# ratschlab/secedo

Hardware: AMD Instinct MI355X
Metric: cell-pair x locus updates/sec (similarity matrix) (higher is better)
Workload: dtype int64; 1 GPU; C3: 8000 cells x 100000 loci; entries=24345058, kept_entries=24223307, reads=23997029, block_cells=128, tiles=2016, normalization=ADD_MIN, max_fragment_length=1000, num_threads=8, parallelism=single GPU, backend=none, world_size=1, rccl_world_size=1

## Files before the change

secedo_amd/csrc/simmat_api.cpp:

```cpp
#include "simmat_handle.hpp"

#include <algorithm>
#include <cstdio>
#include <new>
#include <utility>

using namespace secedo::host;

namespace {

void note_pileup(secedo_simmat *h, uint32_t n_chr, uint64_t n_loci, uint64_t n_entries, const void *read_ids) {
    Fnv1a id;
    for (uint64_t v : {(uint64_t)n_chr, n_loci, n_entries, (uint64_t)reinterpret_cast<uintptr_t>(read_ids)}) id.add(v);
    h->pileup_identity = id.id();
    if (h->override_identity != h->pileup_identity) {
        if (h->pair_bound_override || h->max_shared_override) h->override_dropped = true;
        h->pair_bound_override = 0;
        h->max_shared_override = 0;
        h->override_identity = 0;
    }
}

int check_pileup_args(const secedo_simmat *h, const void *chr_locus_off, const void *locus_entry_off,
                      const void *id_base16, const void *id_base32, const void *group_id_to_pos, uint32_t n_groups) {
    if (!h) return fail(SECEDO_E_INVALID_ARG, "handle is null");
    if (!chr_locus_off || !locus_entry_off) return fail(SECEDO_E_INVALID_ARG, "null offset arrays");
    if ((id_base16 != nullptr) == (id_base32 != nullptr))
        return fail(SECEDO_E_INVALID_ARG, "exactly one of id_base16 / id_base32 must be given");
    if (!group_id_to_pos && n_groups) return fail(SECEDO_E_INVALID_ARG, "group_id_to_pos is null");
    return SECEDO_OK;
}


struct HostPileupStore {
    std::vector<uint32_t> chr, pos, rid, g2p, idb32;
    std::vector<uint64_t> off;
    std::vector<uint16_t> idb16;
};
int fetch_pileup_to_host(const secedo::DeviceFlatPileup &d, hipStream_t s, HostPileupStore *store,
                         secedo::FlatPileupView *v) {
    SECEDO_TRY(hipStreamSynchronize(s));
    auto fetch = [](auto &to, const void *d_src, size_t n) {
        to.resize(n);
        return n ? hipMemcpy(to.data(), d_src, n * sizeof(to[0]), hipMemcpyDeviceToHost) : hipSuccess;
    };
    SECEDO_TRY(fetch(store->chr, d.chr_locus_off, (size_t)d.n_chr + 1));
    SECEDO_TRY(fetch(store->pos, d.locus_pos, d.n_loci));
    SECEDO_TRY(fetch(store->off, d.locus_entry_off, (size_t)d.n_loci + 1));
    SECEDO_TRY(fetch(store->rid, d.read_ids, d.n_entries));
    SECEDO_TRY(fetch(store->g2p, d.group_id_to_pos, d.n_groups));
    if (d.id_base16) SECEDO_TRY(fetch(store->idb16, d.id_base16, d.n_entries));
    else SECEDO_TRY(fetch(store->idb32, d.id_base32, d.n_entries));
    static const uint16_t none16 = 0;
    static const uint32_t none32 = 0;
    *v = secedo::FlatPileupView{store->chr.data(), d.n_chr, store->pos.data(), store->off.data(), store->rid.data(),
                                d.id_base16 ? (store->idb16.empty() ? &none16 : store->idb16.data()) : nullptr,
                                d.id_base16 ? nullptr : (store->idb32.empty() ? &none32 : store->idb32.data()),
                                store->g2p.data(), d.n_groups};
    return SECEDO_OK;
}

int adopt_host_packing(secedo::PackedPileup &from, secedo::DevicePacked *pk) {
    SECEDO_TRY(pk->blk_off.upload(from.blk_off));
    SECEDO_TRY(pk->entry32.upload(from.entry32));
    SECEDO_TRY(pk->mask32.upload(from.mask32));
    SECEDO_TRY(pk->entry.upload(from.entry));
    SECEDO_TRY(pk->entry_read.upload(from.entry_read));
    SECEDO_TRY(pk->range_off.upload(from.range_off));
    SECEDO_TRY(pk->read_off.upload(from.read_off));
    SECEDO_TRY(pk->read_locus.upload(from.read_locus));
    SECEDO_TRY(pk->read_base.upload(from.read_base));
    pk->num_cells = from.num_cells;
    pk->block_cells = from.block_cells;
    pk->num_blocks = from.num_blocks;
    pk->num_loci = from.num_loci;
    pk->num_entries = from.num_entries;
    pk->num_reads = from.num_reads;
    pk->pair_bound = from.pair_bound;
    pk->cell_sq = nullptr;
    pk->cell_sq_n = 0;
    pk->cell_sq_host = std::move(from.cell_sq);
    pk->multi_entries = from.multi_entries;
    pk->max_read_entries = from.max_read_entries;
    pk->n_wide = from.n_wide;
    pk->stage_masks = from.stage_masks;
    pk->count_tile = from.count_tile;
    pk->cap_entries = from.cap_entries;
    pk->cap_loci = from.cap_loci;
    pk->num_ranges = static_cast<uint32_t>(from.range_off.size()) - 1;
    return SECEDO_OK;
}

struct PrepareArgs {
    uint32_t num_cells, max_fragment_length, num_threads, block_cells;
    bool allow_count_tile;
    int mode;
};

int pack_on_device(secedo_simmat *h, const PrepareArgs &p, hipStream_t s, bool *need_host) {
    if (h->have_host) SECEDO_TRY(upload_flat_pileup(h->view, h->raw, &h->dview));
    const std::string err = secedo::pack_pileup_device(h->dview, p.num_cells, p.max_fragment_length, p.num_threads,
                                                       p.block_cells, &secedo::stage_geometry, p.allow_count_tile, s,
                                                       &h->pk, need_host);
    if (!err.empty()) {
        h->have_host = h->have_device = false;
        return fail(err.find("hip") == 0 ? SECEDO_E_HIP : SECEDO_E_INVALID_ARG, err);
    }
    if (*need_host && p.mode == 2) {
        h->have_host = h->have_device = false;
        return fail(SECEDO_E_LIMIT, "this pileup needs the host packing path (a read is longer than "
                                    "max_fragment_length, or a size limit of the device path)");
    }
    if (!*need_host) h->used_device_packing = 1;
    return SECEDO_OK;
}

int pack_on_host(secedo_simmat *h, const PrepareArgs &p, hipStream_t s) {
    HostPileupStore store;
    secedo::FlatPileupView v = h->view;
    if (!h->have_host) SECEDO_CALL(fetch_pileup_to_host(h->dview, s, &store, &v));
    secedo::PackedPileup packed;
    const std::string err = secedo::pack_pileup(v, p.num_cells, p.max_fragment_length, p.num_threads, p.block_cells,
                                                &secedo::stage_geometry, p.allow_count_tile, &packed);
    if (!err.empty()) {
        h->have_host = h->have_device = false;
        return fail(SECEDO_E_INVALID_ARG, err);
    }
    return adopt_host_packing(packed, &h->pk);
}

int build_tile_table(secedo_simmat *h) {
    const uint32_t nb = h->pk.num_blocks;
    if (h->num_tiles == nb * (nb + 1) / 2 && h->tile_row.p) return SECEDO_OK;
    h->num_tiles = nb * (nb + 1) / 2;
    std::vector<uint16_t> trow, tcol;
    trow.reserve(h->num_tiles);
    tcol.reserve(h->num_tiles);
    for (uint32_t i = 0; i < nb; ++i) {
        for (uint32_t j = i; j < nb; ++j) {
            trow.push_back(static_cast<uint16_t>(i));
            tcol.push_back(static_cast<uint16_t>(j));
        }
    }
    SECEDO_TRY(h->tile_row.upload(trow));
    SECEDO_TRY(h->tile_col.upload(tcol));
    h->host_tile_row = trow;
    h->host_tile_col = tcol;
    return SECEDO_OK;
}

int build_flag_lists(secedo_simmat *h, hipStream_t s) {
    const secedo::DevicePacked &pk = h->pk;
    if (!(pk.count_tile && !pk.stage_masks && pk.num_entries)) return SECEDO_OK;
    const uint32_t ne = (uint32_t)pk.num_entries;
    const size_t n_off = (size_t)pk.num_blocks * (pk.num_loci + 1);
    SECEDO_TRY(h->flag_tmp.ensure(secedo::flag_list_scratch_bytes(ne)));
    SECEDO_TRY(h->flag_rec.ensure((size_t)ne * 16));
    SECEDO_TRY(h->flag_idx.ensure((size_t)ne * 4));
    SECEDO_TRY(h->flag_grp.ensure(std::max<size_t>(n_off, 1) * 4));
    SECEDO_TRY(secedo::pack_flag_lists(pk.entry32.as<uint32_t>(), pk.entry.as<uint4>(), ne, pk.blk_off.as<uint32_t>(),
                                       n_off, h->flag_tmp.p, h->flag_grp.as<uint32_t>(), h->flag_rec.as<uint4>(),
                                       h->flag_idx.as<uint32_t>(), s));
    h->flags_ready = true;
    return SECEDO_OK;
}

int print_stamps(secedo_simmat *h) {
    const unsigned long long *counters = h->counters.as<unsigned long long>();
    const bool counts = env_set("SECEDO_STAMPS_COUNTS");
    unsigned long long st[16] = {0};
    SECEDO_TRY(hipMemcpy(st, counters, sizeof(st), hipMemcpyDeviceToHost));
    if (counts) {
        unsigned long long cf[11] = {0};
        SECEDO_TRY(hipMemcpy(cf, counters + 82, sizeof(cf), hipMemcpyDeviceToHost));
        if (cf[0])
            std::fprintf(stderr, "[stamps-correct] pair tests %llu, tail terms %llu, joint terms %llu, later-locus pairs %llu | "
                                 "per wave: pairs phase %.0f cycles (%.0f until the first q records are there), flush phase %.0f cycles, "
                                 "flagged row entries %.0f; busiest lane: %.1f q iterations, %.0f cycles until their records are there\n",
                         cf[0], cf[1], cf[2], cf[3], (double)cf[4] / (double)cf[6], (double)cf[8] / (double)cf[6],
                         (double)cf[5] / (double)cf[6], (double)cf[7] / (double)cf[6], (double)cf[10] / (double)cf[6],
                         (double)cf[9] / (double)cf[6]);
    }
    if (st[8] && counts) {
        const double w = (double)st[8];
        std::fprintf(stderr, "[stamps-counts] sampled waves %llu | per wave cycles: total %.0f barrier-A %.0f stage+barrier-B %.0f "
                             "items(+col prefetch issue) %.0f primary groups %.0f drain %.0f | per primary batch %.0f, per drain batch %.0f "
                             "(%.2f drain batches per primary batch)\n",
                     st[8], st[7] / w, st[2] / w, st[3] / w, st[4] / w, st[5] / w, st[6] / w,
                     (double)st[5] / std::max<double>(1, (double)st[9]), (double)st[6] / std::max<double>(1, (double)st[10]),
                     (double)st[10] / std::max<double>(1, (double)st[9]));
        unsigned long long pw[64] = {0};
        SECEDO_TRY(hipMemcpy(pw, counters + 16, sizeof(pw), hipMemcpyDeviceToHost));
        const double wgs = w / 16.0;
        for (int k = 0; k < 16; ++k)
            std::fprintf(stderr, "[stamps-counts] wave %2d: barrier-A %8.0f  pairs %8.0f  items %8.0f  stage+B %8.0f\n", k,
                         pw[k * 4] / wgs, pw[k * 4 + 1] / wgs, pw[k * 4 + 2] / wgs, pw[k * 4 + 3] / wgs);
    } else if (st[8]) {
        std::fprintf(stderr, "[stamps] waves %llu batches %llu trips %llu | per wave: lifetime %.0f cyc, setup %.0f, "
                             "fill %.0f, trips %.0f | per batch: setup %.0f fill %.0f trips %.0f (%.2f trips)\n",
                     st[8], st[5], st[6], (double)st[7] / st[8], (double)st[2] / st[8], (double)st[3] / st[8],
                     (double)st[4] / st[8], (double)st[2] / st[5], (double)st[3] / st[5], (double)st[4] / st[5],
                     (double)st[6] / st[5]);
        std::fprintf(stderr, "[stamps] per wave: barrier-1 wait %.0f, staging+barrier-2 %.0f, prefetch issue %.0f\n",
                     (double)st[9] / st[8], (double)st[10] / st[8], (double)st[11] / st[8]);
        std::fprintf(stderr, "[stamps] per wave: post-trip %.0f, batch loop total %.0f\n",
                     (double)st[12] / st[8], (double)st[13] / st[8]);
        std::fprintf(stderr, "[stamps] longest wave lifetime %llu cyc; ranges %u workgroups %u\n", st[14],
                     h->pk.num_ranges, h->plan_workgroups);
        std::vector<unsigned long long> wg(std::min<uint32_t>(h->plan_workgroups, 2048u));
        SECEDO_TRY(hipMemcpy(wg.data(), counters + 16, wg.size() * 8, hipMemcpyDeviceToHost));
        std::vector<unsigned long long> det(wg.size() * 8);
        SECEDO_TRY(hipMemcpy(det.data(), counters + 16 + 2048, det.size() * 8, hipMemcpyDeviceToHost));
        for (size_t k = 0; k < wg.size(); ++k)
            std::fprintf(stderr, "[stamps-wg] %zu %llu %llu %llu | hwid %llx ranges %llu listflush %llu endbarrier %llu slab %llu | realbegin %llu realend %llu batchloop %llu\n", k,
                         wg[k] & 0xFFFFFFFFull, (wg[k] >> 32) & 0xFFF, (wg[k] >> 44) & 0xFFF, det[k * 8], det[k * 8 + 1] / 1000,
                         det[k * 8 + 2] / 1000, det[k * 8 + 3] / 1000, det[k * 8 + 4] / 1000, det[k * 8 + 5], det[k * 8 + 6], det[k * 8 + 7] / 1000);
    }
    return SECEDO_OK;
}

}

int secedo::host::set_pileup_view(secedo_simmat *h, const secedo::FlatPileupView &v) {
    SECEDO_CALL(check_pileup_args(h, v.chr_locus_off, v.locus_entry_off, v.id_base16, v.id_base32, v.group_id_to_pos,
                                  v.n_groups));
    h->view = v;
    h->have_host = true;
    h->have_device = false;
    h->prepared = false;
    note_pileup(h, v.n_chr, v.n_loci(), v.n_entries(), v.read_ids);
    return SECEDO_OK;
}

int secedo::host::finalize_mode(secedo_simmat *h, int mode, const int64_t *d_acc, uint32_t row_begin, uint32_t row_end,
                                double *d_out, void *stream, bool keep_max) {
    SECEDO_CALL(check_ready(h, true, d_acc && d_out));
    SECEDO_CALL(check_row_range(h, row_begin, row_end));
    SECEDO_TRY(hipSetDevice(h->device));
    SECEDO_TRY(secedo::launch_finalize(d_acc, h->tile_row.as<uint16_t>(), h->tile_col.as<uint16_t>(), h->num_tiles,
                                       h->pk.num_cells, h->pk.block_cells, h->scale_log2, mode,
                                       h->max_bits.as<unsigned long long>(), row_begin, row_end, d_out,
                                       static_cast<hipStream_t>(stream), keep_max));
    return SECEDO_OK;
}

extern "C" {

const char *secedo_simmat_last_error(void) { return g_error.c_str(); }

const char *secedo_simmat_version(void) { return "secedo-simmat-mi355x 0.1 (gfx950)"; }

int secedo_simmat_device_count(void) {
    int n = 0;
    if (hipGetDeviceCount(&n) != hipSuccess) return 0;
    return n;
}

int secedo_simmat_normalization_from_string(const char *name) {
    if (name) {
        if (!std::strcmp(name, "ADD_MIN")) return SECEDO_NORM_ADD_MIN;
        if (!std::strcmp(name, "EXPONENTIATE")) return SECEDO_NORM_EXPONENTIATE;
        if (!std::strcmp(name, "SCALE_MAX_1")) return SECEDO_NORM_SCALE_MAX_1;
    }
    return fail(SECEDO_E_INVALID_NORMALIZATION,
                std::string("Invalid normalization: ") + (name ? name : "(null)"));
}

double secedo_simmat_llr(uint32_t x_s, uint32_t x_d, double eps, double h, double theta) {
    if (x_s + x_d >= 1 && !secedo::llr_exact_mode()) return secedo::reference_llr_any(eps, h, theta, x_s, x_d, 8);
    return secedo::llr(secedo::make_llr_model(eps, h, theta), x_s, x_d);
}

double secedo_simmat_llr_closed_form(uint32_t x_s, uint32_t x_d, double eps, double h, double theta) {
    return secedo::llr(secedo::make_llr_model(eps, h, theta), x_s, x_d);
}

int secedo_simmat_create(secedo_simmat_t **handle, int device_id) {
    if (!handle) return fail(SECEDO_E_INVALID_ARG, "handle is null");
    *handle = nullptr;
    const int n = secedo_simmat_device_count();
    if (n <= 0) return no_device("the similarity-matrix path");
    if (device_id < 0 || device_id >= n) return fail(SECEDO_E_NO_DEVICE, "device id out of range");
    SECEDO_TRY(hipSetDevice(device_id));
    secedo_simmat *h = new (std::nothrow) secedo_simmat();
    if (!h) return fail(SECEDO_E_LIMIT, "out of host memory");
    h->device = device_id;
    hipError_t e = hipEventCreate(&h->ev_begin);
    if (e == hipSuccess) e = hipEventCreate(&h->ev_end);
    if (e == hipSuccess) e = hipEventCreate(&h->ev_mid);
    if (e != hipSuccess) {
        delete h;
        return fail(SECEDO_E_HIP, std::string("hipEventCreate: ") + hipGetErrorString(e));
    }
    *handle = h;
    return SECEDO_OK;
}

void secedo_simmat_destroy(secedo_simmat_t *h) {
    if (!h) return;
    (void)hipSetDevice(h->device);
    if (h->ev_begin) (void)hipEventDestroy(h->ev_begin);
    if (h->ev_end) (void)hipEventDestroy(h->ev_end);
    if (h->ev_mid) (void)hipEventDestroy(h->ev_mid);
    h->uploads.destroy();
    delete h;
}

int secedo_simmat_set_pileup(secedo_simmat_t *h, const uint32_t *chr_locus_off, uint32_t n_chr,
                             const uint32_t *locus_pos, const uint64_t *locus_entry_off,
                             const uint32_t *read_ids, const uint16_t *id_base16,
                             const uint32_t *id_base32, const uint32_t *group_id_to_pos,
                             uint32_t n_groups) {
    return set_pileup_view(h, secedo::FlatPileupView{chr_locus_off, n_chr, locus_pos, locus_entry_off, read_ids,
                                                     id_base16, id_base32, group_id_to_pos, n_groups});
}

int secedo_simmat_set_pileup_device(secedo_simmat_t *h, const uint32_t *d_chr_locus_off, uint32_t n_chr,
                                    const uint32_t *d_locus_pos, const uint64_t *d_locus_entry_off,
                                    const uint32_t *d_read_ids, const uint16_t *d_id_base16,
                                    const uint32_t *d_id_base32, const uint32_t *d_group_id_to_pos,
                                    uint32_t n_groups, uint32_t n_loci, uint64_t n_entries) {
    SECEDO_CALL(check_pileup_args(h, d_chr_locus_off, d_locus_entry_off, d_id_base16, d_id_base32, d_group_id_to_pos,
                                  n_groups));
    h->dview = make_device_view(d_chr_locus_off, n_chr, d_locus_pos, d_locus_entry_off, d_read_ids, d_id_base16,
                                d_id_base32, d_group_id_to_pos, n_groups, n_loci, n_entries);
    h->have_device = true;
    h->have_host = false;
    h->prepared = false;
    note_pileup(h, n_chr, n_loci, n_entries, d_read_ids);
    return SECEDO_OK;
}

int secedo_simmat_set_packing(secedo_simmat_t *h, int mode) {
    if (!h) return fail(SECEDO_E_INVALID_ARG, "handle is null");
    if (mode < 0 || mode > 2) return fail(SECEDO_E_INVALID_ARG, "packing mode must be 0 (auto), 1 (host) or 2 (device)");
    h->packing_mode = mode;
    return SECEDO_OK;
}

int secedo_simmat_used_device_packing(const secedo_simmat_t *h) { return h ? h->used_device_packing : 0; }

int secedo_simmat_prepare(secedo_simmat_t *h, uint32_t num_cells, uint32_t max_fragment_length,
                          uint32_t num_threads, uint32_t block_cells, void *stream) {
    if (!h) return fail(SECEDO_E_INVALID_ARG, "handle is null");
    if (!h->have_host && !h->have_device) return fail(SECEDO_E_STATE, "set_pileup was not called");
    if (block_cells == 0) {
        const int v = env_int("SECEDO_BLOCK_CELLS", 0);
        if (v == 64 || v == 128) block_cells = static_cast<uint32_t>(v);
    }
    PrepareArgs p{num_cells, max_fragment_length, num_threads, block_cells, env_enabled("SECEDO_COUNT_TILE"),
                  h->packing_mode};
    if (env_is("SECEDO_PACKING", "host")) p.mode = 1;
    if (env_is("SECEDO_PACKING", "device")) p.mode = 2;
    SECEDO_TRY(hipSetDevice(h->device));
    hipStream_t s = static_cast<hipStream_t>(stream);
    h->prepared = false;
    h->used_device_packing = 0;
    h->num_threads = num_threads;

    bool need_host = (p.mode == 1);
    if (!need_host) SECEDO_CALL(pack_on_device(h, p, s, &need_host));
    if (need_host) SECEDO_CALL(pack_on_host(h, p, s));
    h->have_host = h->have_device = false;

    SECEDO_CALL(build_tile_table(h));
    SECEDO_TRY(h->counters.ensure((16 + 2048 * 9) * sizeof(unsigned long long)));
    SECEDO_TRY(h->max_bits.ensure(sizeof(unsigned long long)));
    SECEDO_TRY(hipMemsetAsync(h->counters.p, 0, 16 * sizeof(unsigned long long), s));
    h->prepared = true;
    h->timed = false;
    h->flags_ready = false;
    h->wide_known = false;
    return build_flag_lists(h, s);
}

uint32_t secedo_simmat_num_tiles(const secedo_simmat_t *h) { return h ? h->num_tiles : 0; }
uint32_t secedo_simmat_block_cells(const secedo_simmat_t *h) { return h ? h->pk.block_cells : 0; }
uint64_t secedo_simmat_acc_elems(const secedo_simmat_t *h) {
    return h ? static_cast<uint64_t>(h->num_tiles) * h->pk.block_cells * h->pk.block_cells : 0;
}
uint64_t secedo_simmat_num_entries(const secedo_simmat_t *h) { return h ? h->pk.num_entries : 0; }
uint64_t secedo_simmat_num_reads(const secedo_simmat_t *h) { return h ? h->pk.num_reads : 0; }
uint64_t secedo_simmat_num_loci(const secedo_simmat_t *h) { return h ? h->pk.num_loci : 0; }

uint64_t secedo_simmat_pair_bound(const secedo_simmat_t *h) { return h ? h->pk.pair_bound : 0; }
int secedo_simmat_scale_log2(const secedo_simmat_t *h) { return h ? h->scale_log2 : 0; }
uint32_t secedo_simmat_max_read_entries(const secedo_simmat_t *h) { return h ? h->pk.max_read_entries : 0; }
int secedo_simmat_set_scale_bounds(secedo_simmat_t *h, uint64_t pair_bound, uint32_t max_read_entries) {
    if (!h) return fail(SECEDO_E_INVALID_ARG, "handle is null");
    h->pair_bound_override = pair_bound;
    h->max_shared_override = max_read_entries;
    h->override_identity = (pair_bound || max_read_entries) ? h->pileup_identity : 0;
    h->override_dropped = false;
    return SECEDO_OK;
}
int secedo_simmat_scale_bounds_state(const secedo_simmat_t *h) {
    if (!h) return 0;
    if ((h->pair_bound_override || h->max_shared_override) && h->override_identity == h->pileup_identity) return 1;
    return h->override_dropped ? 2 : 0;
}
int secedo_simmat_set_pair_bound(secedo_simmat_t *h, uint64_t pair_bound) {
    return secedo_simmat_set_scale_bounds(h, pair_bound, h ? h->max_shared_override : 0);
}
int secedo_simmat_cell_squares(secedo_simmat_t *h, uint64_t *d_out, void *stream) {
    SECEDO_CALL(check_ready(h, false, d_out));
    SECEDO_TRY(hipSetDevice(h->device));
    hipStream_t s = static_cast<hipStream_t>(stream);
    const size_t n = h->pk.num_cells;
    SECEDO_TRY(hipMemsetAsync(d_out, 0, n * 8, s));
    if (h->pk.cell_sq && h->pk.cell_sq_n) {
        SECEDO_TRY(hipMemcpyAsync(d_out, h->pk.cell_sq, std::min<size_t>(n, h->pk.cell_sq_n) * 8, hipMemcpyDeviceToDevice, s));
    } else if (!h->pk.cell_sq_host.empty()) {
        SECEDO_TRY(hipMemcpyAsync(d_out, h->pk.cell_sq_host.data(), std::min(n, h->pk.cell_sq_host.size()) * 8,
                                  hipMemcpyHostToDevice, s));
        SECEDO_TRY(hipStreamSynchronize(s));
    }
    return SECEDO_OK;
}

int secedo_simmat_zero_acc(secedo_simmat_t *h, int64_t *d_acc, void *stream) {
    SECEDO_CALL(check_ready(h, false, d_acc));
    SECEDO_TRY(hipSetDevice(h->device));
    SECEDO_TRY(hipMemsetAsync(d_acc, 0, secedo_simmat_acc_elems(h) * sizeof(int64_t),
                              static_cast<hipStream_t>(stream)));
    return SECEDO_OK;
}

int secedo_simmat_tiles_of_rows(const secedo_simmat_t *h, uint32_t row_begin, uint32_t row_end, uint32_t *tile_ids,
                                uint32_t *n_tile_ids) {
    SECEDO_CALL(check_ready(h, false, n_tile_ids));
    SECEDO_CALL(check_row_range(h, row_begin, row_end));
    uint32_t n = 0;
    if (row_begin < row_end) {
        const uint32_t B = h->pk.block_cells, b0 = row_begin / B, b1 = (row_end - 1) / B;
        for (uint32_t t = 0; t < h->num_tiles; ++t) {
            const uint32_t I = h->host_tile_row[t], J = h->host_tile_col[t];
            if ((I >= b0 && I <= b1) || (J >= b0 && J <= b1)) {
                if (tile_ids) tile_ids[n] = t;
                ++n;
            }
        }
    }
    *n_tile_ids = n;
    return SECEDO_OK;
}

int secedo_simmat_max_of_tiles(secedo_simmat_t *h, const int64_t *d_acc, const uint32_t *tile_ids, uint32_t n_tile_ids,
                               double *max_value, void *stream) {
    SECEDO_CALL(check_ready(h, true, d_acc && max_value && (tile_ids || !n_tile_ids)));
    for (uint32_t k = 0; k < n_tile_ids; ++k)
        if (tile_ids[k] >= h->num_tiles) return fail(SECEDO_E_INVALID_ARG, "tile id outside [0, num_tiles)");
    SECEDO_TRY(hipSetDevice(h->device));
    hipStream_t s = static_cast<hipStream_t>(stream);
    DevBuf ids;
    SECEDO_TRY(ids.ensure((size_t)std::max(n_tile_ids, 1u) * 4));
    if (n_tile_ids) SECEDO_TRY(hipMemcpyAsync(ids.p, tile_ids, (size_t)n_tile_ids * 4, hipMemcpyHostToDevice, s));
    SECEDO_TRY(secedo::launch_tile_max(d_acc, h->tile_row.as<uint16_t>(), h->tile_col.as<uint16_t>(), ids.as<uint32_t>(),
                                       n_tile_ids, h->pk.block_cells, h->scale_log2, h->max_bits.as<unsigned long long>(),
                                       s));
    unsigned long long bits = 0;
    SECEDO_TRY(hipMemcpyAsync(&bits, h->max_bits.p, 8, hipMemcpyDeviceToHost, s));
    SECEDO_TRY(hipStreamSynchronize(s));
    std::memcpy(max_value, &bits, 8);
    return SECEDO_OK;
}

int secedo_simmat_finalize_rows_max(secedo_simmat_t *h, int normalization, const int64_t *d_acc, uint32_t row_begin,
                                    uint32_t row_end, double max_value, double *d_out_rows, void *stream) {
    SECEDO_CALL(check_normalization(normalization));
    SECEDO_CALL(check_ready(h, true, d_acc && d_out_rows));
    SECEDO_CALL(check_row_range(h, row_begin, row_end));
    if (!(max_value >= 0.0)) return fail(SECEDO_E_INVALID_ARG, "max_value must be the (non-negative) maximum of D");
    SECEDO_TRY(hipSetDevice(h->device));
    hipStream_t s = static_cast<hipStream_t>(stream);
    unsigned long long bits;
    std::memcpy(&bits, &max_value, 8);
    SECEDO_TRY(hipMemcpyAsync(h->max_bits.p, &bits, 8, hipMemcpyHostToDevice, s));
    SECEDO_TRY(hipStreamSynchronize(s));
    SECEDO_TRY(secedo::launch_finalize(d_acc, h->tile_row.as<uint16_t>(), h->tile_col.as<uint16_t>(), h->num_tiles,
                                       h->pk.num_cells, h->pk.block_cells, h->scale_log2, normalization,
                                       h->max_bits.as<unsigned long long>(), row_begin, row_end, d_out_rows, s, true));
// ... 76 lines not shown
```

secedo_amd/csrc/simmat_kernels.hip:

```cpp
#include "simmat_kernels.hpp"

#include <hip/hip_runtime.h>

#include <algorithm>
#include <type_traits>

namespace secedo {

uint32_t counts_split(uint32_t n_tiles);

namespace {

constexpr uint32_t META_PREV_OVF = 1u << 19;
constexpr uint32_t META_NEXT_OVF = 1u << 20;
constexpr uint32_t C_CELL = 127u;
constexpr uint32_t C_BASE_SHIFT = 7;
constexpr uint32_t C_TAIL = 1u << 9;
constexpr uint32_t C_MULTI = 1u << 10;
constexpr uint32_t C_WIDE = 1u << 11;
constexpr int LUT_DIM = 129;
constexpr int SLUT_DIM = 10;
constexpr long long NO_PAIR = (long long)0x8000000000000000ull;

__device__ __forceinline__ double log_add(double a, double b) {
// ... 1315 lines not shown
                        for (uint32_t base = 0; base < cw; base += 64u) {
                            uint2 w2[GROUP];
                            w2[0] = sJ[min(j0w + base + lane, (uint32_t)CAPJ - 1u)];
#pragma unroll
                            for (int u = 1; u < GROUP; ++u) w2[u] = w2[0];
                            const uint32_t c1 = base + lane < cw ? 1u : 0u;
                            if (DIAG) pair_group(std::true_type{}, itw, xw, yw, w2, c1);
                            else pair_group(std::false_type{}, itw, xw, yw, w2, c1);
                        }
                    }
                    if (c >= IT_WIDE) item[k] = 0u;
                }
            }
            if (r + 1 < r_end) prefetch(r + 1);
            {
                uint2 wc[GROUP], wn[GROUP];
                group_load(item[0], wc);
#pragma unroll
                for (int k = 0; k < JPT; ++k) {
                    if (k + 1 < JPT) group_load(item[k + 1], wn);
                    while (ring_tail - ring_head > (uint32_t)(RING - 64)) drain_one();
                    group_pair(item[k], ix[k], iy[k], wc);
#pragma unroll
                    for (int u = 0; u < GROUP; ++u) wc[u] = wn[u];
                }
            }
            if (r + 1 < r_end) prefetch_rows();
            while (ring_tail != ring_head) drain_one();
        } else {
            if (r + 1 < r_end) {
                prefetch(r + 1);
                prefetch_rows();
            }
            const long long d10 = a.lut[1 * LUT_DIM + 0], d01 = a.lut[0 * LUT_DIM + 1];
            uint32_t upd = 0, skipped = 0;
            for (uint32_t e1 = ib + tid; e1 < ie; e1 += THREADS) {
                const uint32_t r1 = a.entry32[e1];
                const uint32_t l = la + (r1 >> 16);
                const uint32_t j0 = DIAG ? e1 + 1 : offJ[l];
                const uint32_t j1 = offJ[l + 1];
                const uint32_t row = (r1 & C_CELL) * B;
                for (uint32_t e2 = j0; e2 < j1; ++e2) {
                    const uint32_t r2 = a.entry32[e2];
                    const uint32_t x = r1 ^ r2, both = r1 & r2;
                    if (DIAG && (x & C_CELL) == 0u) continue;
                    if (both & C_TAIL) continue;
                    if ((r1 | r2) & C_WIDE) continue;
                    ++upd;
                    long long v = (x & (3u << C_BASE_SHIFT)) ? d01 : d10;
                    if (both & C_MULTI) {
                        v = pair_value_full(a.slow, e1, e2);
                        if (v == NO_PAIR) {
                            ++skipped;
                            continue;
                        }
                    }
                    atomicAdd(&dst[row + (r2 & C_CELL)], (unsigned long long)v);
                }
            }
            n_updates += upd;
            n_pairs += (unsigned long long)upd - skipped;
        }
        n_updates += upd_lane;
        n_pairs += add_lane;
    }
    __syncthreads();

    {
        unsigned long long *out = reinterpret_cast<unsigned long long *>(a.slab) + (size_t)blockIdx.x * B * B;
        for (uint32_t i = tid; i < B * B; i += THREADS) out[i] = tile64[(i / B) * ROW_Q + (i % B)];
    }
    for (int off = 32; off > 0; off >>= 1) {
        n_updates += __shfl_down(n_updates, off);
        n_pairs += __shfl_down(n_pairs, off);
    }
    unsigned long long *red = reinterpret_cast<unsigned long long *>(sJ);
    if (lane == 0u) {
        red[(tid >> 6) * 2] = n_updates;
        red[(tid >> 6) * 2 + 1] = n_pairs;
    }
    __syncthreads();
    if (tid == 0u) {
        unsigned long long u = 0, q = 0;
        for (int w = 0; w < WAVES; ++w) {
            u += red[w * 2];
            q += red[w * 2 + 1];
        }
        if (u | q) {
            atomicAdd(&a.counters[0], u);
            atomicAdd(&a.counters[1], q);
        }
    }
}

__global__ __launch_bounds__(256) void k_masks_words(const uint32_t *entry32, const uint32_t *mask32, uint32_t n,
                                                    uint32_t *y, uint32_t *xcol, uint32_t *xrow) {
    for (uint32_t d = blockIdx.x * 256 + threadIdx.x; d < n; d += gridDim.x * 256) {
        const uint32_t e = entry32[d], m = mask32[d];
        const uint32_t f = masks_flags(e, m);
        y[d] = masks_planes(m);
        xcol[d] = f | ((e & C_CELL) << 3);
        xrow[d] = f | MX_DEAD | ((m >> 8) & 0xFFu);
    }
}

__global__ __launch_bounds__(256) void k_wide_count(const uint32_t *entry32, const uint32_t *blk_off, uint32_t stride,
                                                   uint32_t *cnt) {
    const uint32_t b = blockIdx.y, e0 = blk_off[(size_t)b * stride], e1 = blk_off[(size_t)b * stride + stride - 1u];
    uint32_t n = 0;
    for (uint32_t d = e0 + blockIdx.x * 256 + threadIdx.x; d < e1; d += gridDim.x * 256) n += (entry32[d] & C_WIDE) ? 1u : 0u;
    for (int off = 32; off > 0; off >>= 1) n += __shfl_down(n, off);
    if ((threadIdx.x & 63u) == 0u && n) atomicAdd(&cnt[b], n);
}
__global__ __launch_bounds__(1024) void k_wide_scan(const uint32_t *cnt, uint32_t nb, uint32_t *off, uint32_t *cur) {
    __shared__ uint32_t s[1024];
    const uint32_t tid = threadIdx.x;
    s[tid] = tid < nb ? cnt[tid] : 0u;
    __syncthreads();
    for (uint32_t d = 1; d < 1024; d <<= 1) {
        const uint32_t v = tid >= d ? s[tid - d] : 0u;
        __syncthreads();
        s[tid] += v;
        __syncthreads();
    }
    if (tid < nb) {
        const uint32_t ex = s[tid] - cnt[tid];
        off[tid] = ex;
        cur[tid] = ex;
    }
    if (tid == nb - 1u) off[nb] = s[tid];
}
__global__ __launch_bounds__(256) void k_wide_fill(const uint32_t *entry32, const uint32_t *blk_off, uint32_t stride,
                                                  uint32_t *cur, uint32_t *list) {
    const uint32_t b = blockIdx.y, e0 = blk_off[(size_t)b * stride], e1 = blk_off[(size_t)b * stride + stride - 1u];
    for (uint32_t d = e0 + blockIdx.x * 256 + threadIdx.x; d < e1; d += gridDim.x * 256)
        if (entry32[d] & C_WIDE) list[atomicAdd(&cur[b], 1u)] = d;
}

struct WideArgs {
    const uint32_t *blk_off;
    uint32_t stride;
    const uint32_t *entry32;
    const uint4 *entry;
    const SlowPathArgs *slow;
    const long long *lut;
    const uint16_t *tile_row, *tile_col;
    uint32_t tile_begin;
    const uint32_t *tile_ids;
    const uint32_t *wide_off, *wide_list;
    long long *acc;
    unsigned long long *counters;
};
template <int B>
__global__ __launch_bounds__(256) void wide_pairs(const WideArgs a) {
    const uint32_t t = a.tile_ids ? a.tile_ids[blockIdx.x] : a.tile_begin + blockIdx.x;
    const uint32_t I = a.tile_row[t], J = a.tile_col[t];
    const bool diag = I == J;
    const long long d10 = a.lut[1 * LUT_DIM + 0], d01 = a.lut[0 * LUT_DIM + 1];
    unsigned long long *dst = reinterpret_cast<unsigned long long *>(a.acc) + (size_t)t * B * B;
    uint32_t upd = 0, skipped = 0;
    for (int side = 0; side < (diag ? 1 : 2); ++side) {
        const uint32_t bw = side ? J : I, bo = side ? I : J;
        const uint32_t *off_o = a.blk_off + (size_t)bo * a.stride;
        for (uint32_t k = a.wide_off[bw] + (threadIdx.x >> 6); k < a.wide_off[bw + 1]; k += 4) {
            const uint32_t ew = a.wide_list[k];
            const uint32_t rw = a.entry32[ew];
            const uint32_t l = a.entry[ew].w;
            for (uint32_t eo = off_o[l] + (threadIdx.x & 63u); eo < off_o[l + 1]; eo += 64u) {
                const uint32_t ro = a.entry32[eo];
                if (ro & C_WIDE) {
                    if (side == 1) continue;
                    if (diag && eo <= ew) continue;
                } else if (diag && eo == ew) {
                    continue;
                }
                const uint32_t x = rw ^ ro, both = rw & ro;
                if (diag && (x & C_CELL) == 0u) continue;
                if (both & C_TAIL) continue;
                ++upd;
                long long v = (x & (3u << C_BASE_SHIFT)) ? d01 : d10;
                const uint32_t e_row = side ? eo : ew, e_col = side ? ew : eo;
                if (both & C_MULTI) {
                    v = pair_value_full(a.slow, e_row, e_col);
                    if (v == NO_PAIR) {
                        ++skipped;
                        continue;
                    }
                }
                const uint32_t r_row = side ? ro : rw, r_col = side ? rw : ro;
                atomicAdd(&dst[(r_row & C_CELL) * B + (r_col & C_CELL)], (unsigned long long)v);
            }
        }
    }
    unsigned long long u = upd, q = (unsigned long long)upd - skipped;
    for (int off = 32; off > 0; off >>= 1) {
        u += __shfl_down(u, off);
        q += __shfl_down(q, off);
    }
    if ((threadIdx.x & 63u) == 0u && (u | q)) {
        atomicAdd(&a.counters[0], u);
        atomicAdd(&a.counters[1], q);
    }
}

constexpr uint32_t kJointOwned = 1u << 31;
__device__ __forceinline__ uint32_t joint_pack(bool owned, uint32_t xs, uint32_t xd) {
    return (owned ? kJointOwned : 0u) | (xs << 15) | xd;
}
__device__ __noinline__ uint32_t joint_counts_walk(const SlowPathArgs *sp, const uint32_t *flag_idx, uint32_t locus,
                                                   uint32_t i1, uint32_t i2) {
    const uint32_t r1 = sp->entry_read[flag_idx[i1]], r2 = sp->entry_read[flag_idx[i2]];
    uint32_t j1 = sp->read_off[r1], e1 = sp->read_off[r1 + 1];
    uint32_t j2 = sp->read_off[r2], e2 = sp->read_off[r2 + 1];
    uint32_t xs = 0, xd = 0, first = 0xFFFFFFFFu;
    while (j1 < e1 && j2 < e2) {
        const uint32_t l1 = sp->read_locus[j1], l2 = sp->read_locus[j2];
        if (l1 == l2) {
            if (first == 0xFFFFFFFFu) first = l1;
            if (sp->read_base[j1] == sp->read_base[j2]) ++xs; else ++xd;
            ++j1; ++j2;
        } else if (l1 < l2) {
            ++j1;
        } else {
            ++j2;
        }
    }
    return joint_pack(first == locus, xs, xd);
}

__device__ __forceinline__ uint32_t joint_counts(const SlowPathArgs *sp, const uint32_t *flag_idx, const uint4 A1,
                                                 const uint4 A2, uint32_t i1, uint32_t i2) {
    if (A1.y & A2.y & 0xFFFFu) return 0u;
    const bool same = (((A1.x ^ A2.x) >> 16) & 3u) == 0u;
    if ((A1.x & A2.x & (META_PREV_OVF | META_NEXT_OVF)) == 0u) {
        const uint32_t shared = (A1.y & A2.y) >> 16;
        const uint32_t x = A1.z ^ A2.z;
        const uint32_t diff = ((x & 0xFFFFu) | (x >> 16)) & shared;
        const uint32_t nd = __popc(diff);
        return joint_pack(true, __popc(shared) - nd + (same ? 1u : 0u), nd + (same ? 0u : 1u));
    }
    return joint_counts_walk(sp, flag_idx, A1.w, i1, i2);
}

struct CorrectArgs {
    const uint32_t *blk_off;
    uint32_t stride;
    const uint32_t *flag_grp;
    const uint4 *flag_rec;
    const uint32_t *flag_idx;
    const SlowPathArgs *slow;
    const long long *lut;
    const uint16_t *tile_row, *tile_col;
    uint32_t tile_begin;
    const uint32_t *tile_ids;
    const void *slab;
    const uint32_t *tile_wg_begin;
    int64_t *acc;
    unsigned long long *counters;
    uint32_t split;
    uint32_t overwrite;
    unsigned long long *max_bits;
    double max_scale;
};

__host__ __device__ inline CorrectArgs correct_args(const AccumulateArgs &args) {
    CorrectArgs c = {};
    c.blk_off = args.blk_off;
    c.stride = args.stride;
    c.flag_grp = args.flag_grp;
    c.flag_rec = args.flag_rec;
    c.flag_idx = args.flag_idx;
    c.slow = args.slow;
    c.lut = args.lut;
    c.tile_row = args.tile_row;
    c.tile_col = args.tile_col;
    c.tile_begin = args.tile_begin;
    c.tile_ids = args.tile_ids;
    c.slab = args.slab;
    c.tile_wg_begin = args.tile_wg_begin;
    c.acc = args.acc;
    c.counters = args.counters;
    c.max_scale = args.max_scale;
    return c;
}

template <int B, int THREADS>
__device__ __forceinline__ void correct_setup(const long long *lut, long long d10, long long d01,
                                              unsigned long long *corr, long long *scorr) {
    const uint32_t tid = threadIdx.x;
    for (uint32_t i = tid; i < (uint32_t)(B * B); i += THREADS) corr[i] = 0ull;
    if (tid < (uint32_t)(SLUT_DIM * SLUT_DIM)) {
        const uint32_t xs = tid / SLUT_DIM, xd = tid % SLUT_DIM;
        scorr[tid] = lut[xs * LUT_DIM + xd] - (long long)xs * d10 - (long long)xd * d01;
    }
    __syncthreads();
}

template <int B, int THREADS, int NPRE, bool IN_CORR>
__device__ __forceinline__ void correct_tile(const CorrectArgs &a, unsigned long long *corr, const long long *scorr,
                                             long long *part, uint32_t t_local, uint32_t part_id, uint32_t t,
                                             long long d10, long long d01, const uint32_t (&pre)[NPRE],
                                             bool prefetched) {
    constexpr int U = 6;
    const uint32_t tid = threadIdx.x, lane = tid & 63u;
    const uint32_t S = a.split;
    const uint32_t I = a.tile_row[t], J = a.tile_col[t];
    const bool diag = I == J;
    long long upd_delta = 0, pair_delta = 0;
#ifdef SECEDO_STAMPS
    unsigned long long dg_tests = 0, dg_tail = 0, dg_joint = 0, dg_later = 0;
    long long dg_loads = 0, dg_qwait = 0, dg_qiter = 0;
    uint32_t dg_sink = 0;
    const long long dg_t0 = __builtin_readcyclecounter();
#endif
    const size_t rowI = (size_t)I * a.stride, rowJ = (size_t)J * a.stride;
    const uint32_t p0 = a.flag_grp[rowI], p1 = a.flag_grp[rowI + a.stride - 1u];
    for (uint32_t base = p0 + part_id * (uint32_t)(THREADS * U); base < p1; base += S * (uint32_t)(THREADS * U)) {
        uint4 A1[U];
        uint32_t qa[U], qb[U];
#ifdef SECEDO_STAMPS
        const long long dg_b0 = __builtin_readcyclecounter();
#endif
#pragma unroll
        for (int u = 0; u < U; ++u) {
            const uint32_t p = base + (uint32_t)u * THREADS + tid;
            A1[u] = p < p1 ? a.flag_rec[p] : make_uint4(0, 0, 0, 0);
        }
#pragma unroll
        for (int u = 0; u < U; ++u) {
            const uint32_t p = base + (uint32_t)u * THREADS + tid;
            const size_t g = rowJ + A1[u].w;
            qa[u] = p < p1 ? a.flag_grp[g] : 0u;
            qb[u] = p < p1 ? a.flag_grp[g + 1] : 0u;
            if (diag) qa[u] = p + 1u;
        }
#ifdef SECEDO_STAMPS
        dg_sink += qa[0] + qb[U - 1];
        const long long dg_b1 = __builtin_readcyclecounter();
        dg_loads += dg_b1 - dg_b0;
#endif
        auto pair_pq = [&](const uint4 P, uint32_t p, const uint4 Q, uint32_t q) {
            const uint32_t row1 = (P.x & 0xFFFFu) - I * B, row2 = (Q.x & 0xFFFFu) - J * B;
            if (diag && row1 == row2) return;
#ifdef SECEDO_STAMPS
            ++dg_tests;
#endif
            const bool multi1 = P.y != 0u || (P.x & (META_PREV_OVF | META_NEXT_OVF)) != 0u;
            const bool tails = (P.x & Q.x & (1u << 18)) != 0u;
            const bool multi2 = Q.y != 0u || (Q.x & (META_PREV_OVF | META_NEXT_OVF)) != 0u;
            if (!tails && !(multi1 && multi2)) return;
            unsigned long long *cell = &corr[row1 * B + row2];
            const bool same = (((P.x ^ Q.x) >> 16) & 3u) == 0u;
            if (tails) {
                atomicAdd(cell, (unsigned long long)(-(same ? d10 : d01)));
                --upd_delta;
                --pair_delta;
#ifdef SECEDO_STAMPS
                ++dg_tail;
#endif
                return;
            }
            const uint32_t jc = joint_counts(a.slow, a.flag_idx, P, Q, p, q);
            const uint32_t xs = (jc >> 15) & 0xFFFFu, xd = jc & 0x7FFFu;
            if ((jc & kJointOwned) == 0u) {
                --pair_delta;
#ifdef SECEDO_STAMPS
                ++dg_later;
#endif
                return;
            }
            if (xs + xd < 2u) return;
            long long term;
            if (xs < (uint32_t)SLUT_DIM && xd < (uint32_t)SLUT_DIM) {
                term = scorr[xs * SLUT_DIM + xd];
            } else {
                const long long joint = xs + xd <= REF_TABLE_MAX
                        ? a.lut[xs * LUT_DIM + xd] : llr_fixed_device(a.slow, xs, xd, P.x & 0xFFFFu, Q.x & 0xFFFFu);
                term = joint - (long long)xs * d10 - (long long)xd * d01;
            }
            atomicAdd(cell, (unsigned long long)term);
#ifdef SECEDO_STAMPS
            ++dg_joint;
#endif
        };
        static_assert(U % 2 == 0, "lists in pairs");
#pragma unroll
        for (int u = 0; u < U; u += 2) {
            const uint32_t pA = base + (uint32_t)u * THREADS + tid, pB = pA + THREADS;
            uint32_t qA = qa[u], qB = qa[u + 1];
            const uint32_t eA = qb[u], eB = qb[u + 1];
            while (qA < eA || qB < eB) {
                const bool hA = qA < eA, hB = qB < eB;
                uint4 QA = make_uint4(0, 0, 0, 0), QB = make_uint4(0, 0, 0, 0);
                if (hA) QA = a.flag_rec[qA];
                if (hB) QB = a.flag_rec[qB];
#ifdef SECEDO_STAMPS
                ++dg_qiter;
#endif
                if (hA) pair_pq(A1[u], pA, QA, qA);
                if (hB) pair_pq(A1[u + 1], pB, QB, qB);
                qA += hA ? 1u : 0u;
                qB += hB ? 1u : 0u;
            }
        }
    }
    for (int off = 32; off > 0; off >>= 1) {
        upd_delta += __shfl_down(upd_delta, off);
        pair_delta += __shfl_down(pair_delta, off);
    }
    if (lane == 0u) {
        part[(tid >> 6) * 2] = upd_delta;
        part[(tid >> 6) * 2 + 1] = pair_delta;
    }
#ifdef SECEDO_STAMPS
    for (int off = 32; off > 0; off >>= 1) {
        dg_tests += __shfl_down(dg_tests, off);
        dg_tail += __shfl_down(dg_tail, off);
        dg_joint += __shfl_down(dg_joint, off);
        dg_later += __shfl_down(dg_later, off);
    }
    for (int off = 32; off > 0; off >>= 1) {
        dg_qwait = max(dg_qwait, (long long)__shfl_down(dg_qwait, off));
        dg_qiter = max(dg_qiter, (long long)__shfl_down(dg_qiter, off));
    }
    __shared__ unsigned long long dg_part[4];
    if (tid < 4u) dg_part[tid] = 0ull;
    __syncthreads();
    if (lane == 0u) {
        atomicAdd(&dg_part[0], dg_tests);
        atomicAdd(&dg_part[1], dg_tail);
        atomicAdd(&dg_part[2], dg_joint);
        atomicAdd(&dg_part[3], dg_later);
    }
    const long long dg_t1 = __builtin_readcyclecounter();
#endif
    __syncthreads();
    if (tid == 0u) {
        long long u = 0, q = 0;
        for (int w = 0; w < THREADS / 64; ++w) {
            u += part[2 * w];
            q += part[2 * w + 1];
        }
        if (u) atomicAdd(&a.counters[0], (unsigned long long)u);
        if (q) atomicAdd(&a.counters[1], (unsigned long long)q);
    }
    const uint32_t w0 = a.tile_wg_begin[t_local], w1 = a.tile_wg_begin[t_local + 1];
    long long *dst = reinterpret_cast<long long *>(a.acc) + (size_t)t * B * B;
    long long best = 0;
    constexpr int F = (B * B / THREADS) < 8 ? (B * B / THREADS) : 8;
    static_assert((B * B) % (THREADS * F) == 0, "whole batches");
    const uint32_t *slab32 = reinterpret_cast<const uint32_t *>(a.slab);
    int batch = 0;
    for (uint32_t c0 = tid; c0 < (uint32_t)(B * B); c0 += THREADS * F, ++batch) {
        uint32_t n_same[F], n_diff[F];
        long long old[F];
#pragma unroll
        for (int f = 0; f < F; ++f) {
            n_same[f] = 0;
            n_diff[f] = 0;
            old[f] = (S == 1u && !a.overwrite) ? dst[c0 + f * THREADS] : 0ll;
        }
        if (prefetched) {
#pragma unroll
            for (int f = 0; f < F; ++f) {
                uint32_t v = 0;
#pragma unroll
                for (int k = 0; k < NPRE; ++k) v = (k == batch * F + f) ? pre[k] : v;
                n_same[f] = v & 0xFFFFu;
                n_diff[f] = v >> 16;
            }
        }
        for (uint32_t w = (prefetched || IN_CORR) ? w1 : w0; w < w1; ++w) {
#pragma unroll
            for (int f = 0; f < F; ++f) {
                const uint32_t c = c0 + f * THREADS;
                if (S == 1u || (c / THREADS) % S == part_id) {
                    const uint32_t v = slab32[(size_t)w * B * B + c];
                    n_same[f] += v & 0xFFFFu;
                    n_diff[f] += v >> 16;
                }
            }
        }
#pragma unroll
        for (int f = 0; f < F; ++f) {
            const uint32_t c = c0 + f * THREADS;
            const long long sum = (long long)corr[c] + (long long)n_same[f] * d10 + (long long)n_diff[f] * d01;
            if (S == 1u) {
                if (sum || a.overwrite) dst[c] = old[f] + sum;
                if (a.max_bits) {
                    if (diag) corr[c] = (unsigned long long)(old[f] + sum);
                    else best = max(best, old[f] + sum);
                }
            } else if (sum) {
                atomicAdd(reinterpret_cast<unsigned long long *>(&dst[c]), (unsigned long long)sum);
            }
        }
    }
    if (a.max_bits) {
        if (diag) {
            __syncthreads();
            for (uint32_t c = tid; c < (uint32_t)(B * B); c += THREADS) {
                const uint32_t r = c / B, col = c % B;
                if (r < col) best = max(best, (long long)corr[c] + (long long)corr[col * B + r]);
            }
        }
        for (int off = 32; off > 0; off >>= 1) best = max(best, (long long)__shfl_down(best, off));
        __syncthreads();
        if (lane == 0u) part[tid >> 6] = best;
        __syncthreads();
        if (tid == 0u) {
            for (int w = 1; w < THREADS / 64; ++w) best = max(best, part[w]);
            atomicMax(a.max_bits, (unsigned long long)__double_as_longlong((double)best * a.max_scale));
        }
    }
#ifdef SECEDO_STAMPS
    if (tid == 0u) {
        atomicAdd(&a.counters[82], dg_part[0]);
        atomicAdd(&a.counters[83], dg_part[1]);
        atomicAdd(&a.counters[84], dg_part[2]);
        atomicAdd(&a.counters[85], dg_part[3]);
        atomicAdd(&a.counters[86], (unsigned long long)(dg_t1 - dg_t0));
        atomicAdd(&a.counters[87], (unsigned long long)(__builtin_readcyclecounter() - dg_t1));
        atomicAdd(&a.counters[88], 1ull);
        atomicAdd(&a.counters[89], (unsigned long long)(p1 - p0));
        atomicAdd(&a.counters[90], (unsigned long long)dg_loads + (dg_sink == 0xFFFFFFFFu ? 1ull : 0ull));
        atomicAdd(&a.counters[91], (unsigned long long)dg_qwait);
        atomicAdd(&a.counters[92], (unsigned long long)dg_qiter);
    }
#endif
}


template <int B, int THREADS>
__global__ __launch_bounds__(THREADS) void correct_tiles(const CorrectArgs a) {
    extern __shared__ unsigned long long corr[];
    __shared__ long long part[2 * (THREADS / 64)];
    __shared__ long long scorr[SLUT_DIM * SLUT_DIM];
    const uint32_t tid = threadIdx.x;
    const uint32_t S = a.split, t_local = blockIdx.x / S, part_id = blockIdx.x % S;
    const uint32_t t = a.tile_ids ? a.tile_ids[t_local] : a.tile_begin + t_local;
    const long long d10 = a.lut[1 * LUT_DIM + 0], d01 = a.lut[0 * LUT_DIM + 1];
    correct_setup<B, THREADS>(a.lut, d10, d01, corr, scorr);
    constexpr int PRE = (B * B) / THREADS, NPRE = PRE <= 16 ? PRE : 1;
    const bool prefetched = S == 1u && a.tile_wg_begin[t_local + 1] - a.tile_wg_begin[t_local] == 1u && PRE <= 16;
    uint32_t pre[NPRE];
    if (prefetched) {
        const uint32_t *src = reinterpret_cast<const uint32_t *>(a.slab) + (size_t)a.tile_wg_begin[t_local] * B * B;
#pragma unroll
        for (int k = 0; k < NPRE; ++k) pre[k] = __builtin_nontemporal_load(&src[tid + (uint32_t)k * THREADS]);
    }
    correct_tile<B, THREADS, NPRE, false>(a, corr, scorr, part, t_local, part_id, t, d10, d01, pre, prefetched);
}

template <int B, int THREADS, int NCNT>
__device__ __forceinline__ void correct_epilogue(const AccumulateArgs &a, unsigned char *lds, uint32_t t_local,
                                                 const uint32_t (&cnt)[NCNT]) {
    unsigned long long *corr = reinterpret_cast<unsigned long long *>(lds);
    long long *scorr = reinterpret_cast<long long *>(lds + (size_t)B * B * 8);
    long long *part = scorr + SLUT_DIM * SLUT_DIM;
    const uint32_t tid = threadIdx.x;
    const long long d10 = a.lut[1 * LUT_DIM + 0], d01 = a.lut[0 * LUT_DIM + 1];
#pragma unroll
    for (int k = 0; k < NCNT; ++k)
        corr[tid + (uint32_t)k * THREADS] = (unsigned long long)((long long)(cnt[k] & 0xFFFFu) * d10
                                                                 + (long long)(cnt[k] >> 16) * d01);
    if (tid < (uint32_t)(SLUT_DIM * SLUT_DIM)) {
        const uint32_t xs = tid / SLUT_DIM, xd = tid % SLUT_DIM;
        scorr[tid] = a.lut[xs * LUT_DIM + xd] - (long long)xs * d10 - (long long)xd * d01;
    }
    __syncthreads();
    CorrectArgs c = correct_args(a);
    c.split = 1u;
    c.overwrite = a.overwrite ? 1u : 0u;
    c.max_bits = a.max_bits;
    const uint32_t none[1] = {0u};
    const uint32_t t = a.tile_ids ? a.tile_ids[t_local] : a.tile_begin + t_local;
    correct_tile<B, THREADS, 1, true>(c, corr, scorr, part, t_local, 0u, t, d10, d01, none, false);
}

template <int B>
__global__ __launch_bounds__(256) void reduce_slabs(const void *slab, const uint32_t *tile_wg_begin,
                                                   uint32_t tile_begin, const uint32_t *tile_ids,
                                                   const long long *lut, long long *acc) {
    const uint32_t t_local = blockIdx.x / (B * B / 256);
    const uint32_t cell = (blockIdx.x % (B * B / 256)) * 256 + threadIdx.x;
    const uint32_t w0 = tile_wg_begin[t_local], w1 = tile_wg_begin[t_local + 1];
    long long sum = 0;
    const long long *p = reinterpret_cast<const long long *>(slab) + cell;
    for (uint32_t w = w0; w < w1; ++w) sum += p[(size_t)w * B * B];
    long long *dst = &acc[(size_t)(tile_ids ? tile_ids[t_local] : tile_begin + t_local) * B * B + cell];
    if (sum) *dst += sum;
}

template <int B>
__global__ __launch_bounds__(256) void reduce_max(const long long *acc, const uint16_t *tile_row,
                                                  const uint16_t *tile_col, const uint32_t *tile_ids,
                                                  uint32_t n_tiles, double scale, unsigned long long *out_bits) {
    const size_t total = (size_t)n_tiles * B * B;
    long long best = 0;
    for (size_t idx = (size_t)blockIdx.x * 256 + threadIdx.x; idx < total; idx += (size_t)gridDim.x * 256) {
        const uint32_t rc = (uint32_t)(idx % (B * B));
        const uint32_t t = tile_ids ? tile_ids[idx / (B * B)] : (uint32_t)(idx / (B * B));
        long long v = acc[(size_t)t * B * B + rc];
        if (tile_row[t] == tile_col[t]) {
            const uint32_t r = rc / B, c = rc % B;
            v = r < c ? v + acc[(size_t)t * B * B + c * B + r] : 0;
        }
        best = max(best, v);
    }
    for (int off = 32; off > 0; off >>= 1) best = max(best, (long long)__shfl_down(best, off));
    __shared__ long long part[4];
    if ((threadIdx.x & 63) == 0) part[threadIdx.x >> 6] = best;
    __syncthreads();
    if (threadIdx.x == 0) {
        best = max(max(part[0], part[1]), max(part[2], part[3]));
        atomicMax(out_bits, (unsigned long long)__double_as_longlong((double)best * scale));
    }
}

template <int B>
__global__ __launch_bounds__(256) void write_matrix(const long long *acc, const uint16_t *tile_row,
                                                    const uint16_t *tile_col, uint32_t n, double scale, int mode,
                                                    const unsigned long long *max_bits, uint32_t row_begin,
                                                    uint32_t row_end, double *out) {
    constexpr uint32_t SB = 32, PER = B / SB;
    __shared__ double V[SB][SB + 1];
    const uint32_t t = blockIdx.x / (PER * PER), sub = blockIdx.x % (PER * PER);
    const uint32_t a = sub / PER, b = sub % PER;
    const uint32_t I = tile_row[t], J = tile_col[t];
    const bool diag = (I == J);
    if (diag && a > b) return;
    const double mx = (mode == 0 || mode == 2) ? __longlong_as_double((long long)*max_bits) : 0.0;
    const double add = fabs(-mx);
    const double inv = 1.0 / mx;
    const long long *tile = acc + (size_t)t * B * B;
    const uint32_t tx = threadIdx.x % SB, ty = threadIdx.x / SB;
    const uint32_t i0 = I * B + a * SB, j0 = J * B + b * SB;
    if ((i0 >= row_end || i0 + SB <= row_begin) && (j0 >= row_end || j0 + SB <= row_begin)) return;
#pragma unroll
    for (uint32_t k = 0; k < SB; k += 8) {
        const uint32_t r = ty + k, c = tx;
        long long v = tile[(a * SB + r) * B + b * SB + c];
        if (diag) v += tile[(b * SB + c) * B + a * SB + r];
        const double d = (double)v * scale;
        double w;
        switch (mode) {
            case 0: w = (d * -1.0) + add; break;
            case 1: w = 1.0 / (exp(d) + 1.0); break;
            case 2: w = d * inv; break;
            default: w = d; break;
        }
        if (i0 + r == j0 + c) w = 0.0;
        V[r][c] = w;
        const uint32_t i = i0 + r;
        if (i < n && j0 + c < n && i >= row_begin && i < row_end) out[(size_t)(i - row_begin) * n + j0 + c] = w;
    }
    if (diag && a == b) return;
    __syncthreads();
#pragma unroll
    for (uint32_t k = 0; k < SB; k += 8) {
        const uint32_t c = ty + k, r = tx;
        const uint32_t j = j0 + c;
        if (i0 + r < n && j < n && j >= row_begin && j < row_end) out[(size_t)(j - row_begin) * n + i0 + r] = V[r][c];
    }
}

template <int B, int THREADS, int CAPJ, int CAPL, int HCAP, bool MASKS>
hipError_t launch_acc(const AccumulateArgs &args, uint32_t grid, hipStream_t stream) {
    constexpr size_t lds = (size_t)B * B * 8 + (size_t)CAPJ * 2 + ((size_t)CAPL + 2) * 2
            + (MASKS ? (size_t)CAPJ * 4 + SLUT_DIM * SLUT_DIM * 8 : 0) + 16
            + (size_t)(THREADS / 64) * ((size_t)HCAP + 64 * 8 + (MASKS ? 64 * 4 : 0)
                                        + (size_t)joint_list_cap<B, THREADS, CAPJ, CAPL, HCAP, MASKS>() * 10);
    static_assert(lds <= 160 * 1024, "LDS budget");
    static_assert((CAPL + 2) % 4 == 0 && CAPJ % 8 == 0 && HCAP % 16 == 0, "alignment of the LDS carve-up");
    auto kern = &accumulate_tiles<B, THREADS, CAPJ, CAPL, HCAP, MASKS>;
    static thread_local int configured_device = -1;
    int dev = 0;
    hipError_t e = hipGetDevice(&dev);
    if (e != hipSuccess) return e;
    if (configured_device != dev) {
        e = hipFuncSetAttribute(reinterpret_cast<const void *>(kern), hipFuncAttributeMaxDynamicSharedMemorySize,
                                (int)lds);
        if (e != hipSuccess) return e;
        configured_device = dev;
    }
    hipLaunchKernelGGL(kern, dim3(grid), dim3(THREADS), lds, stream, args);
    hipLaunchKernelGGL((reduce_slabs<B>), dim3(args.n_tiles * (B * B / 256)), dim3(256), 0, stream,
                       args.slab, args.tile_wg_begin, args.tile_begin, args.tile_ids, args.lut,
                       reinterpret_cast<long long *>(args.acc));
    return hipGetLastError();
}

template <int B>
hipError_t launch_correct(const AccumulateArgs &args, hipStream_t stream);

template <int B, int THREADS, int CAPJ, int CAPL, int GROUP>
hipError_t launch_masks(const AccumulateArgs &args, uint32_t grid, hipStream_t stream) {
    constexpr size_t lds = (size_t)B * MASKS_ROW_Q(B) * 8 + (size_t)CAPJ * 8 + ((size_t)CAPL + 2) * 2
            + MLUT_WORDS * 8 + (size_t)(THREADS / 64) * MASKS_RING * 12;
    static_assert(lds <= 80 * 1024, "two workgroups per CU");
    static_assert((CAPL + 2) % 4 == 0 && CAPJ % 8 == 0, "alignment of the LDS carve-up");
    auto kern = &accumulate_masks<B, THREADS, CAPJ, CAPL, GROUP>;
    static thread_local int configured_device = -1;
    int dev = 0;
    hipError_t e = hipGetDevice(&dev);
// ... 217 lines not shown
```

Measured before the change: 758.7 billion updates/s.

## Load-balance pair loop across wave lanes via prefix-sum and binary-search redistribution

Replaces the per-lane while loop over each thread's q-range with wave-cooperative work distribution. A wave-level inclusive scan of per-lane pair counts is built, and each lane then picks pairs from the flattened range using a binary search through ds_bpermute, fetching the owning P record by permute. This is meant to remove divergence where the busiest lane dictates how long the wave runs. It adds scan and bpermute overhead per batch and unrolls three rounds of 64 pairs at a time.

Result: no change. 759.1 billion updates/s, median of 3 (+0.1%).

```diff
diff --git a/secedo_amd/csrc/simmat_api.cpp b/secedo_amd/csrc/simmat_api.cpp
--- a/secedo_amd/csrc/simmat_api.cpp
+++ b/secedo_amd/csrc/simmat_api.cpp
@@ -176,7 +176,7 @@
         if (cf[0])
             std::fprintf(stderr, "[stamps-correct] pair tests %llu, tail terms %llu, joint terms %llu, later-locus pairs %llu | "
                                  "per wave: pairs phase %.0f cycles (%.0f until the first q records are there), flush phase %.0f cycles, "
-                                 "flagged row entries %.0f; busiest lane: %.1f q iterations, %.0f cycles until their records are there\n",
+                                 "flagged row entries %.0f; %.1f rounds of 64 pairs per wave, %.0f cycles until their records are there\n",
                          cf[0], cf[1], cf[2], cf[3], (double)cf[4] / (double)cf[6], (double)cf[8] / (double)cf[6],
                          (double)cf[5] / (double)cf[6], (double)cf[7] / (double)cf[6], (double)cf[10] / (double)cf[6],
                          (double)cf[9] / (double)cf[6]);
diff --git a/secedo_amd/csrc/simmat_kernels.hip b/secedo_amd/csrc/simmat_kernels.hip
--- a/secedo_amd/csrc/simmat_kernels.hip
+++ b/secedo_amd/csrc/simmat_kernels.hip
@@ -1641,6 +1641,7 @@
                                              long long d10, long long d01, const uint32_t (&pre)[NPRE],
                                              bool prefetched) {
     constexpr int U = 6;
+    constexpr int R = 3;
     const uint32_t tid = threadIdx.x, lane = tid & 63u;
     const uint32_t S = a.split;
     const uint32_t I = a.tile_row[t], J = a.tile_col[t];
@@ -1678,6 +1679,22 @@
         const long long dg_b1 = __builtin_readcyclecounter();
         dg_loads += dg_b1 - dg_b0;
 #endif
+        uint32_t Px[U], Py[U], Pz[U], incl[U], qoff[U];
+#pragma unroll
+        for (int u = 0; u < U; ++u) {
+            const uint32_t len = qb[u] > qa[u] ? qb[u] - qa[u] : 0u;
+            uint32_t s = len;
+#pragma unroll
+            for (uint32_t d = 1; d < 64u; d <<= 1) {
+                const uint32_t up = (uint32_t)__shfl_up((int)s, d);
+                s += lane >= d ? up : 0u;
+            }
+            incl[u] = s;
+            qoff[u] = qa[u] - (s - len);
+            Px[u] = A1[u].x;
+            Py[u] = A1[u].y;
+            Pz[u] = A1[u].z;
+        }
         auto pair_pq = [&](const uint4 P, uint32_t p, const uint4 Q, uint32_t q) {
             const uint32_t row1 = (P.x & 0xFFFFu) - I * B, row2 = (Q.x & 0xFFFFu) - J * B;
             if (diag && row1 == row2) return;
@@ -1722,24 +1739,55 @@
             ++dg_joint;
 #endif
         };
-        static_assert(U % 2 == 0, "lists in pairs");
-#pragma unroll
-        for (int u = 0; u < U; u += 2) {
-            const uint32_t pA = base + (uint32_t)u * THREADS + tid, pB = pA + THREADS;
-            uint32_t qA = qa[u], qB = qa[u + 1];
-            const uint32_t eA = qb[u], eB = qb[u + 1];
-            while (qA < eA || qB < eB) {
-                const bool hA = qA < eA, hB = qB < eB;
-                uint4 QA = make_uint4(0, 0, 0, 0), QB = make_uint4(0, 0, 0, 0);
-                if (hA) QA = a.flag_rec[qA];
-                if (hB) QB = a.flag_rec[qB];
+#pragma unroll 1
+        for (int u = 0; u < U; ++u) {
+            const uint32_t cx = Px[0], cy = Py[0], cz = Pz[0], ci = incl[0], co = qoff[0];
+#pragma unroll
+            for (int k = 0; k + 1 < U; ++k) {
+                Px[k] = Px[k + 1];
+                Py[k] = Py[k + 1];
+                Pz[k] = Pz[k + 1];
+                incl[k] = incl[k + 1];
+                qoff[k] = qoff[k + 1];
+            }
+            const uint32_t T = (uint32_t)__builtin_amdgcn_readlane((int)ci, 63);
+            const uint32_t pw = base + (uint32_t)u * THREADS + (tid - lane);
+            for (uint32_t j0 = 0; j0 < T; j0 += 64u * R) {
+                uint4 Q[R];
+                uint32_t own[R], qi[R];
+#pragma unroll
+                for (int r = 0; r < R; ++r) {
+                    Q[r] = make_uint4(0, 0, 0, 0);
+                    own[r] = 0u;
+                    qi[r] = 0u;
+                    if (j0 + 64u * r < T) {
+                        const uint32_t j = j0 + 64u * r + lane;
+                        uint32_t lo = 0u;
+#pragma unroll
+                        for (uint32_t s = 32u; s > 0u; s >>= 1) {
+                            const uint32_t v = (uint32_t)__builtin_amdgcn_ds_bpermute((int)((lo + s - 1u) << 2), (int)ci);
+                            lo += v <= j ? s : 0u;
+                        }
+                        own[r] = lo;
+                        qi[r] = (uint32_t)__builtin_amdgcn_ds_bpermute((int)(lo << 2), (int)co) + j;
+                        if (j < T) Q[r] = a.flag_rec[qi[r]];
 #ifdef SECEDO_STAMPS
-                ++dg_qiter;
+                        ++dg_qiter;
 #endif
-                if (hA) pair_pq(A1[u], pA, QA, qA);
-                if (hB) pair_pq(A1[u + 1], pB, QB, qB);
-                qA += hA ? 1u : 0u;
-                qB += hB ? 1u : 0u;
+                    }
+                }
+#pragma unroll
+                for (int r = 0; r < R; ++r) {
+                    if (j0 + 64u * r < T) {
+                        const int src = (int)(own[r] << 2);
+                        uint4 P;
+                        P.x = (uint32_t)__builtin_amdgcn_ds_bpermute(src, (int)cx);
+                        P.y = (uint32_t)__builtin_amdgcn_ds_bpermute(src, (int)cy);
+                        P.z = (uint32_t)__builtin_amdgcn_ds_bpermute(src, (int)cz);
+                        P.w = Q[r].w;
+                        if (j0 + 64u * r + lane < T) pair_pq(P, pw + own[r], Q[r], qi[r]);
+                    }
+                }
             }
         }
     }
```
